# shenyunhang/NA-fWebSOD

Measured on AMD Instinct MI355X. Metric: images/sec (600px, 2000 proposals) VGG16-C5 WSDDN fwd+bwd, higher is better.
Workload: dtype f32 (2xf16 split, 3-pass f16 MFMA, fp32 accumulate)

## Files before the change

### include/naws.h

```cpp
#ifndef NAWS_H_
#define NAWS_H_

#include <stdint.h>

#ifdef __cplusplus
extern "C" {
#endif

#define NAWS_OK 0
#define NAWS_ERR_SHAPE (-1)
#define NAWS_ERR_ARG (-2)
#define NAWS_ERR_NULL (-3)
#define NAWS_ERR_LAUNCH (-4)
#define NAWS_ERR_UNSUPPORTED (-5)

#define NAWS_LAYOUT_NCHW 0
#define NAWS_LAYOUT_NHWC 1

const char* naws_version(void);
int naws_last_hip_error(void);


int naws_conv3x3_c3_nchw_to_nhwc_fwd(const float* X, const float* Wt, const float* bias,
                                     int N, int H, int W, int Cout, int relu,
                                     float* Y, void* stream);

int naws_conv3x3_pack_weight(const float* W_oihw, int Cout, int Cin, float* W_packed,
                             void* stream);

int naws_conv3x3_nhwc_fwd(const float* X, const float* Wp, const float* bias,
                          int N, int H, int W, int Cin, int Cout, int dilation, int relu,
                          float* Y, void* stream);

int64_t naws_winograd_workspace_floats(int N, int H, int W, int Cin, int Cout, int dilation);
int naws_winograd_weight_transform(const float* W_oihw, int Cout, int Cin, float* U,
                                   void* stream);
int naws_conv3x3_winograd_nhwc_fwd(const float* X, const float* U, const float* bias,
                                   int N, int H, int W, int Cin, int Cout, int dilation, int relu,
                                   float* workspace, float* Y, void* stream);

int naws_maxpool2x2_nhwc_fwd(const float* X, int N, int H, int W, int C, int stride,
                             float* Y, void* stream);

int naws_maxpool3x3_nhwc_fwd(const float* X, int N, int H, int W, int C, int stride,
                             float* Y, void* stream);

int naws_nchw_to_nhwc(const float* X, int N, int C, int H, int W, float* Y, void* stream);
int naws_nhwc_to_nchw(const float* X, int N, int H, int W, int C, float* Y, void* stream);
// ... 417 lines not shown
```

### na-fwebsod_amd/csrc/misc_ops.hip

```cpp
#include <float.h>
#include <math.h>
#include "naws_common.h"

thread_local int g_naws_last_hip_error = 0;

extern "C" const char* naws_version(void) { return "naws-hip 0.1 (gfx950)"; }
extern "C" int naws_last_hip_error(void) { return g_naws_last_hip_error; }

#include <atomic>
#include <mutex>
#include <string.h>
namespace {
constexpr int LDS_SLOTS = 512;
constexpr int MAX_DEV = 256;
struct LdsSlot {
  std::atomic<const void*> kernel;
  std::atomic<unsigned long long> dev[MAX_DEV / 64];
};
LdsSlot g_lds_slots[LDS_SLOTS];
std::mutex g_lds_mutex;
std::atomic<int> g_knobs[NAWS_KNOB_COUNT] = {{0}, {0}, {0}, {11}, {0}, {42}, {0}, {0}, {0}};
const char* const g_knob_names[NAWS_KNOB_COUNT] = {"gemm", "x3", "h2", "conv_ring", "conv_bn",
                                                    "roi_nw", "wino", "split", "sgd_wgs"};
}

int naws_allow_lds_impl(const void* kernel, int bytes) {
  int dev = 0;
  if (hipGetDevice(&dev) != hipSuccess) return naws_check_launch();
  const bool in_range = dev >= 0 && dev < MAX_DEV;
  const size_t h0 = ((uintptr_t)kernel >> 4) % LDS_SLOTS;
  if (in_range) {
    size_t h = h0;
    for (int probe = 0; probe < LDS_SLOTS; ++probe, h = (h + 1) % LDS_SLOTS) {
      const void* k = g_lds_slots[h].kernel.load(std::memory_order_acquire);
      if (k == kernel) {
        if ((g_lds_slots[h].dev[dev >> 6].load(std::memory_order_acquire) >> (dev & 63)) & 1ULL)
          return NAWS_OK;
        break;
      }
      if (k == nullptr) break;
    }
  }
  std::lock_guard<std::mutex> lock(g_lds_mutex);
  LdsSlot* slot = nullptr;
  if (in_range) {
    size_t h = h0;
// ... 161 lines not shown
#pragma unroll
    for (int k = 0; k < 27; ++k) {
      const float v = in[k];
      const float* wr = wl + k * Cout + g * OC_PER;
#pragma unroll
      for (int o = 0; o < OC_PER; ++o) acc[o] = fmaf(v, wr[o], acc[o]);
    }
    float* out = Y + pix * Cout + g * OC_PER;
#pragma unroll
    for (int o = 0; o < OC_PER; o += 4) {
      float4 r;
      r.x = acc[o + 0] + bl[g * OC_PER + o + 0];
      r.y = acc[o + 1] + bl[g * OC_PER + o + 1];
      r.z = acc[o + 2] + bl[g * OC_PER + o + 2];
      r.w = acc[o + 3] + bl[g * OC_PER + o + 3];
      if (relu) { r.x = fmaxf(r.x, 0.f); r.y = fmaxf(r.y, 0.f); r.z = fmaxf(r.z, 0.f); r.w = fmaxf(r.w, 0.f); }
      *reinterpret_cast<float4*>(out + o) = r;
    }
  }
}


constexpr int C3_TW = 64, C3_TH = 8, C3_STRIP = 32, C3_LD = C3_TW + 4;
__global__ __launch_bounds__(256) void conv_c3_tile_kernel(const float* __restrict__ X,
                                                           const float* __restrict__ Wt,
                                                           const float* __restrict__ bias, int H,
                                                           int W, int relu, float* __restrict__ Y) {
  __shared__ float tile[3][C3_TH + 2][C3_LD];
  __shared__ __attribute__((aligned(16))) float wl[27][64];
  const int x0 = blockIdx.x * C3_TW, y0 = blockIdx.y * C3_TH, n = blockIdx.z;
  const float* Xn = X + (int64_t)n * 3 * H * W;
  for (int i = threadIdx.x; i < 3 * (C3_TH + 2) * (C3_TW + 2); i += 256) {
    const int col = i % (C3_TW + 2);
    const int r = (i / (C3_TW + 2)) % (C3_TH + 2);
    const int c = i / ((C3_TW + 2) * (C3_TH + 2));
    const int yy = y0 + r - 1, xx = x0 + col - 1;
    const bool ok = (yy >= 0) && (yy < H) && (xx >= 0) && (xx < W);
    const int yc = min(max(yy, 0), H - 1), xc = min(max(xx, 0), W - 1);
    const float v = Xn[((int64_t)c * H + yc) * W + xc];
    tile[c][r][col] = ok ? v : 0.f;
  }
  for (int i = threadIdx.x; i < 27 * 64; i += 256) wl[i % 27][i / 27] = Wt[i];
  __syncthreads();
  const int q = threadIdx.x & 15, grp = threadIdx.x >> 4;
  const int row = grp & 7, strip = grp >> 3;
  float w[27][4];
#pragma unroll
  for (int k = 0; k < 27; ++k) {
    const float4 t = *reinterpret_cast<const float4*>(&wl[k][4 * q]);
    w[k][0] = t.x; w[k][1] = t.y; w[k][2] = t.z; w[k][3] = t.w;
  }
  float4 bv = make_float4(0.f, 0.f, 0.f, 0.f);
  if (bias) bv = *reinterpret_cast<const float4*>(bias + 4 * q);
  const int y = y0 + row;
  const int cx = strip * C3_STRIP;
  float win[3][3][3];
#pragma unroll
  for (int c = 0; c < 3; ++c)
#pragma unroll
    for (int kh = 0; kh < 3; ++kh) {
      win[c][kh][0] = tile[c][row + kh][cx];
      win[c][kh][1] = tile[c][row + kh][cx + 1];
    }
  float* yrow = Y + (((int64_t)n * H + y) * W + x0 + cx) * 64 + 4 * q;
#pragma unroll
  for (int i = 0; i < C3_STRIP; ++i) {
// ... 33 lines not shown

__global__ __launch_bounds__(TB) void maxpool2_kernel(const float4* __restrict__ X, int N, int H,
                                                      int W, int C4, int stride, int Ho, int Wo,
                                                      float4* __restrict__ Y) {
  const int64_t total = (int64_t)N * Ho * Wo * C4;
  for (int64_t t = (int64_t)blockIdx.x * TB + threadIdx.x; t < total;
       t += (int64_t)gridDim.x * TB) {
    const int c = (int)(t % C4);
    const int xo = (int)((t / C4) % Wo);
    const int yo = (int)((t / ((int64_t)C4 * Wo)) % Ho);
    const int n = (int)(t / ((int64_t)C4 * Wo * Ho));
    const int y = yo * stride, x = xo * stride;
    const float4* p = X + (((int64_t)n * H + y) * W + x) * C4 + c;
    const float4 a = p[0], b = p[C4], d = p[(int64_t)W * C4], e = p[(int64_t)W * C4 + C4];
    float4 r;
    r.x = fmaxf(fmaxf(a.x, b.x), fmaxf(d.x, e.x));
    r.y = fmaxf(fmaxf(a.y, b.y), fmaxf(d.y, e.y));
    r.z = fmaxf(fmaxf(a.z, b.z), fmaxf(d.z, e.z));
    r.w = fmaxf(fmaxf(a.w, b.w), fmaxf(d.w, e.w));
    Y[t] = r;
  }
}

__global__ void transpose_batched_kernel(const float* __restrict__ X, int rows, int cols,
                                         float* __restrict__ Y) {
  __shared__ float tile[32][33];
  const int64_t boff = (int64_t)blockIdx.z * rows * cols;
  const int c0 = blockIdx.x * 32, r0 = blockIdx.y * 32;
  for (int i = threadIdx.y; i < 32; i += blockDim.y) {
    const int r = r0 + i, c = c0 + threadIdx.x;
    if (r < rows && c < cols) tile[i][threadIdx.x] = X[boff + (int64_t)r * cols + c];
  }
  __syncthreads();
  for (int i = threadIdx.y; i < 32; i += blockDim.y) {
    const int c = c0 + i, r = r0 + threadIdx.x;
    if (r < rows && c < cols) Y[boff + (int64_t)c * rows + r] = tile[threadIdx.x][i];
  }
}

__global__ void unary_kernel(int op, const float* __restrict__ X, int64_t n, float a, float b,
                             float* __restrict__ Y) {
  for (int64_t i = (int64_t)blockIdx.x * blockDim.x + threadIdx.x; i < n;
       i += (int64_t)gridDim.x * blockDim.x) {
    const float x = X[i];
    float y;
    switch (op) {
// ... 123 lines not shown
}

__global__ void dropout_mask_kernel(uint64_t seed, uint32_t thr, int64_t n,
                                    float* __restrict__ mask) {
  for (int64_t i = (int64_t)blockIdx.x * blockDim.x + threadIdx.x; i < n;
       i += (int64_t)gridDim.x * blockDim.x)
    mask[i] = naws_keep(seed, (uint64_t)i, thr) ? 1.0f : 0.0f;
}

inline int grid_for(int64_t n, int tb = TB, int cap = 256 * 8) {
  return (int)std::min<int64_t>(std::max<int64_t>(naws_cdiv(n, tb), 1), cap);
}

}

extern "C" int naws_conv3x3_c3_nchw_to_nhwc_fwd(const float* X, const float* Wt,
                                                const float* bias, int N, int H, int W, int Cout,
                                                int relu, float* Y, void* stream) {
  if (N <= 0 || H <= 0 || W <= 0 || Cout <= 0) return NAWS_ERR_SHAPE;
  if (Cout % 16 != 0 || ((uintptr_t)Y % 16) != 0) return NAWS_ERR_ARG;
  NAWS_REQUIRE_PTR(X); NAWS_REQUIRE_PTR(Wt); NAWS_REQUIRE_PTR(Y);
  if (Cout == 64 && N <= 65535 && naws_cdiv(H, C3_TH) <= 65535) {
    dim3 grid((unsigned)naws_cdiv(W, C3_TW), (unsigned)naws_cdiv(H, C3_TH), (unsigned)N);
    hipLaunchKernelGGL(conv_c3_tile_kernel, grid, dim3(256), 0, (hipStream_t)stream, X, Wt, bias,
                       H, W, relu, Y);
    return naws_check_launch();
  }
  const size_t lds = (size_t)(27 + 1) * Cout * sizeof(float);
  const int64_t total = (int64_t)N * H * W * (Cout / 16);
  hipLaunchKernelGGL(conv_c3_kernel<16>, dim3(grid_for(total, TB, 256 * 16)), dim3(TB), lds,
                     (hipStream_t)stream, X, Wt, bias, N, H, W, Cout, relu, Y);
  return naws_check_launch();
}

extern "C" int naws_conv3x3_pack_weight(const float* W_oihw, int Cout, int Cin, float* W_packed,
                                        void* stream) {
  if (Cout <= 0 || Cin <= 0) return NAWS_ERR_SHAPE;
  NAWS_REQUIRE_PTR(W_oihw); NAWS_REQUIRE_PTR(W_packed);
  hipLaunchKernelGGL(pack_weight_kernel, dim3(grid_for((int64_t)Cout * Cin * 9)), dim3(TB), 0,
                     (hipStream_t)stream, W_oihw, Cout, Cin, W_packed);
  return naws_check_launch();
}

extern "C" int naws_maxpool2x2_nhwc_fwd(const float* X, int N, int H, int W, int C, int stride,
                                        float* Y, void* stream) {
  if (N <= 0 || H < 2 || W < 2 || C <= 0) return NAWS_ERR_SHAPE;
  if (stride != 1 && stride != 2) return NAWS_ERR_ARG;
  if (C % 4 != 0 || (((uintptr_t)X | (uintptr_t)Y) % 16) != 0) return NAWS_ERR_ARG;
  NAWS_REQUIRE_PTR(X); NAWS_REQUIRE_PTR(Y);
  const int Ho = (H - 2) / stride + 1, Wo = (W - 2) / stride + 1;
  const int64_t total = (int64_t)N * Ho * Wo * (C / 4);
  hipLaunchKernelGGL(maxpool2_kernel, dim3(grid_for(total, TB, 256 * 16)), dim3(TB), 0,
                     (hipStream_t)stream, (const float4*)X, N, H, W, C / 4, stride, Ho, Wo,
                     (float4*)Y);
  return naws_check_launch();
}

static int transpose_batched(const float* X, int batch, int rows, int cols, float* Y,
                             void* stream) {
  if (batch <= 0 || rows <= 0 || cols <= 0) return NAWS_ERR_SHAPE;
  NAWS_REQUIRE_PTR(X); NAWS_REQUIRE_PTR(Y);
  if (batch > 65535 || naws_cdiv(rows, 32) > 65535) return NAWS_ERR_UNSUPPORTED;
  dim3 grid((unsigned)naws_cdiv(cols, 32), (unsigned)naws_cdiv(rows, 32), batch);
  hipLaunchKernelGGL(transpose_batched_kernel, grid, dim3(32, 8), 0, (hipStream_t)stream, X,
                     rows, cols, Y);
  return naws_check_launch();
}

extern "C" int naws_nchw_to_nhwc(const float* X, int N, int C, int H, int W, float* Y,
                                 void* stream) {
  if (H <= 0 || W <= 0) return NAWS_ERR_SHAPE;
  return transpose_batched(X, N, C, H * W, Y, stream);
}
// ... 184 lines not shown
```

### na-fwebsod_amd/csrc/naws_common.h

```cpp
#pragma once
#include <hip/hip_runtime.h>
#include <stdint.h>
#include <algorithm>
#include "naws.h"

#define NAWS_WAVE 64

extern thread_local int g_naws_last_hip_error;

static inline int naws_check_launch() {
  hipError_t e = hipGetLastError();
  if (e != hipSuccess) {
    g_naws_last_hip_error = (int)e;
    return NAWS_ERR_LAUNCH;
  }
  return NAWS_OK;
}

int naws_allow_lds_impl(const void* kernel, int bytes);
template <typename K>
static inline int naws_allow_lds(K kernel, int bytes = 160 * 1024) {
  return naws_allow_lds_impl(reinterpret_cast<const void*>(kernel), bytes);
}

int naws_wino_col_gemm_impl(int P, int Cout, int Cin, const void* V2, const float* invV,
                            const void* U2, const float* scaleU, float* S, hipStream_t stream);

enum NawsKnob { NAWS_KNOB_GEMM = 0, NAWS_KNOB_X3, NAWS_KNOB_H2, NAWS_KNOB_CONV_RING,
                NAWS_KNOB_CONV_BN, NAWS_KNOB_ROI_NW, NAWS_KNOB_WINO, NAWS_KNOB_SPLIT, NAWS_KNOB_SGD_WGS,
                NAWS_KNOB_COUNT };
int naws_knob(int knob);

#define NAWS_REQUIRE_PTR(p) \
  do {                      \
    if ((p) == nullptr) return NAWS_ERR_NULL; \
  } while (0)

static inline int64_t naws_cdiv(int64_t a, int64_t b) { return (a + b - 1) / b; }

__device__ __forceinline__ float wave_sum(float v) {
#pragma unroll
  for (int o = 32; o > 0; o >>= 1) v += __shfl_xor(v, o, 64);
  return v;
}
__device__ __forceinline__ float wave_max(float v) {
#pragma unroll
  for (int o = 32; o > 0; o >>= 1) v = fmaxf(v, __shfl_xor(v, o, 64));
  return v;
}

__device__ __host__ __forceinline__ uint32_t naws_hash_u32(uint64_t seed, uint64_t idx) {
  uint64_t z = seed + 0x9E3779B97F4A7C15ull * (idx + 1);
// ... 185 lines not shown
```

### na-fwebsod_amd/csrc/roi_ops.hip

```cpp
#include <float.h>
#include <stdlib.h>
#include "naws_common.h"

namespace {

struct RoiBins {
  int batch, start_w, start_h, roi_w, roi_h;
};

__device__ __forceinline__ RoiBins roi_frame(const float* roi, float spatial_scale) {
  RoiBins b;
  b.batch = (int)roi[0];
  int start_w = (int)roundf(roi[1] * spatial_scale);
  int start_h = (int)roundf(roi[2] * spatial_scale);
  int end_w = (int)roundf(roi[3] * spatial_scale);
  int end_h = (int)roundf(roi[4] * spatial_scale);
  b.start_w = start_w;
  b.start_h = start_h;
  b.roi_w = max(end_w - start_w + 1, 1);
  b.roi_h = max(end_h - start_h + 1, 1);
  return b;
}

__device__ __forceinline__ void bin_range(int p, float bin_size, int roi_start, int limit,
// ... 338 lines not shown
  unsigned short* dst = Q + pl * plane_out;
  for (int u = threadIdx.x; u < 512; u += 256) {
    const int hh = u & 1, i = (u >> 1) & 15, sl = u >> 5;
    const int slab = k0 / 16 + sl;
    uint4 v = make_uint4(0u, 0u, 0u, 0u);
    if (slab * 16 < K && r0 + i < R)
      v = *reinterpret_cast<const uint4*>(src + ((long long)slab * R + r0 + i) * 16 + hh * 8);
    unsigned short* d = &t[sl][i][hh * 8];
    d[0] = v.x & 0xffff; d[1] = v.x >> 16; d[2] = v.y & 0xffff; d[3] = v.y >> 16;
    d[4] = v.z & 0xffff; d[5] = v.z >> 16; d[6] = v.w & 0xffff; d[7] = v.w >> 16;
  }
  __syncthreads();
  const int k = k0 + threadIdx.x;
  if (k >= K) return;
  const int sl = threadIdx.x >> 4, kk = threadIdx.x & 15;
  unsigned w[8];
#pragma unroll
  for (int i = 0; i < 8; ++i) w[i] = t[sl][2 * i][kk] | ((unsigned)t[sl][2 * i + 1][kk] << 16);
  unsigned short* o = dst + ((long long)blockIdx.y * K + k) * 16;
  *reinterpret_cast<uint4*>(o) = make_uint4(w[0], w[1], w[2], w[3]);
  *reinterpret_cast<uint4*>(o + 8) = make_uint4(w[4], w[5], w[6], w[7]);
}

template <int STEP>
__global__ __launch_bounds__(256) void roi_maxmap_kernel(const float* __restrict__ S, int H, int W,
                                                         int C, float* __restrict__ D,
                                                         long long total4) {
  const long long i = (long long)blockIdx.x * 256 + threadIdx.x;
  if (i >= total4) return;
  const int c4 = C / 4;
  const int cq = (int)(i % c4);
  const long long pix = i / c4;
  const int x = (int)(pix % W), y = (int)((pix / W) % H);
  const int dy = (y + STEP < H) ? STEP : 0, dx = (x + STEP < W) ? STEP : 0;
  const float* base = S + (pix * C + cq * 4);
  const float4 v00 = *reinterpret_cast<const float4*>(base);
  const float4 v01 = *reinterpret_cast<const float4*>(base + (long long)dx * C);
  const float4 v10 = *reinterpret_cast<const float4*>(base + (long long)dy * W * C);
  const float4 v11 = *reinterpret_cast<const float4*>(base + ((long long)dy * W + dx) * C);
  float4 m = make_float4(-FLT_MAX, -FLT_MAX, -FLT_MAX, -FLT_MAX);
#define NAWS_MX(b, v) \
  b.x = (v.x > b.x) ? v.x : b.x; b.y = (v.y > b.y) ? v.y : b.y; \
  b.z = (v.z > b.z) ? v.z : b.z; b.w = (v.w > b.w) ? v.w : b.w;
  NAWS_MX(m, v00) NAWS_MX(m, v01) NAWS_MX(m, v10) NAWS_MX(m, v11)
#undef NAWS_MX
  *reinterpret_cast<float4*>(D + (pix * C + cq * 4)) = m;
// ... 123 lines not shown
  const long long K = (long long)C * pooled_h * pooled_w;
  if (C % 64 != 0 || pooled_h * pooled_w > 256 || K % 32 != 0 || (int64_t)R * (C / 64) >= 0x7fffffffLL)
    return NAWS_ERR_UNSUPPORTED;
  if ((((uintptr_t)X | (uintptr_t)planes) & 15) != 0) return NAWS_ERR_ARG;
  RoiPlaneOut po;
  po.P = (unsigned short*)planes; po.inv_scale = scales + R; po.amax_words = (const unsigned*)amax_words;
  po.n_words = n_words; po.plane = K * R; po.R = R; po.bf16 = 0;
  hipLaunchKernelGGL(roi_pool_nhwc_xcd_kernel<true>, dim3((unsigned)(R * (C / 64))), dim3(64),
                     (size_t)(64 * pooled_h * pooled_w + 1) * sizeof(float), (hipStream_t)stream, X, C,
                     H, W, rois, R, boost, pooled_h, pooled_w, spatial_scale, C / 64, (float*)nullptr,
                     po);
  return naws_check_launch();
}

extern "C" int64_t naws_roi_pool_workspace_floats(int N, int C, int H, int W) {
  if (N <= 0 || C <= 0 || H <= 0 || W <= 0) return 0;
  return (int64_t)2 * N * H * W * C;
}

static int roi_maxmaps(const float* X, int N, int C, int H, int W, float* M2, float* M4,
                       hipStream_t s) {
  const long long total4 = (long long)N * H * W * (C / 4);
  if (naws_cdiv(total4, 256) > 0x7fffffffLL) return NAWS_ERR_UNSUPPORTED;
  hipLaunchKernelGGL(roi_maxmap_kernel<1>, dim3((unsigned)naws_cdiv(total4, 256)), dim3(256), 0, s, X, H,
                     W, C, M2, total4);
  hipLaunchKernelGGL(roi_maxmap_kernel<2>, dim3((unsigned)naws_cdiv(total4, 256)), dim3(256), 0, s,
                     (const float*)M2, H, W, C, M4, total4);
  return naws_check_launch();
}

extern "C" int naws_roi_pool_f_nhwc_hier_fwd(const float* X, int N, int C, int H, int W,
                                             const float* rois, int R, const float* boost,
                                             int pooled_h, int pooled_w, float spatial_scale,
                                             float* workspace, float* Y, void* stream) {
  if (R < 0 || N <= 0 || C <= 0 || H <= 0 || W <= 0 || pooled_h <= 0 || pooled_w <= 0)
    return NAWS_ERR_SHAPE;
  if (R == 0) return NAWS_OK;
  NAWS_REQUIRE_PTR(X); NAWS_REQUIRE_PTR(rois); NAWS_REQUIRE_PTR(Y); NAWS_REQUIRE_PTR(workspace);
  if (C % 64 != 0 || pooled_h * pooled_w > 256 || (int64_t)R * (C / 64) >= 0x7fffffffLL)
    return NAWS_ERR_UNSUPPORTED;
  if ((((uintptr_t)X | (uintptr_t)workspace) & 15) != 0) return NAWS_ERR_ARG;
  hipStream_t s = (hipStream_t)stream;
  const int rc = roi_maxmaps(X, N, C, H, W, workspace, workspace + (long long)N * H * W * C, s);
  if (rc != NAWS_OK) return rc;
  hipLaunchKernelGGL((roi_pool_nhwc_xcd_kernel<false, true, 4>), dim3((unsigned)(R * (C / 64))), dim3(256),
                     (size_t)(64 * pooled_h * pooled_w + 1) * sizeof(float), s, X, C, H, W, rois, R,
// ... 425 lines not shown
```

### na-fwebsod_amd/naws_hip/engine.py

```python

import collections
import contextlib
import os

import numpy as np
import torch

from . import head_arith
from . import lib as L
from . import ops
from .planes import ALL, FcPlanes
from .reducer import ArenaReducer, message_slice, owner_pieces
from .update import HIDDEN, UpdateSchedule

VGG16_CONVS = [
    ('conv1_1', 3, 64, 1), ('conv1_2', 64, 64, 1), ('pool', 2),
    ('conv2_1', 64, 128, 1), ('conv2_2', 128, 128, 1), ('pool', 2),
    ('conv3_1', 128, 256, 1), ('conv3_2', 256, 256, 1), ('conv3_3', 256, 256, 1), ('pool', 2),
    ('conv4_1', 256, 512, 1), ('conv4_2', 512, 512, 1), ('conv4_3', 512, 512, 1), ('pool4',),
    ('conv5_1', 512, 512, None), ('conv5_2', 512, 512, None), ('conv5_3', 512, 512, None),
]

ConvStep = collections.namedtuple('ConvStep',
                                  'name form cin cout dilation direct_alt pool2 weight_bound')
# ... 180 lines not shown
            wd.append(w)
        if any(e % 4 for e in ends):
            raise NotImplementedError('SGD hyper-parameter runs must end on multiples of 4 floats')
        self._seg_host = (list(ends), list(lr_mult), list(wd))
        self.seg_end = torch.tensor(ends, dtype=torch.int64, device=device)
        self.seg_lr_mult = torch.tensor(lr_mult, dtype=torch.float32, device=device)
        self.seg_wd = torch.tensor(wd, dtype=torch.float32, device=device)
        self.lr = torch.zeros((1,), dtype=torch.float32, device=device)
        self._lr_host = 0.0
        self.sgd_iter_count = 0
        self.step_count = 0
        self.conv_layers = []
        self.stat_state = None
        self.conv_streams = True
        self.fused_planes = True
        self.fuse_wgrad_update = True
        self.defer_update = None
        self.DIRECT_MIN_TILES = 256
        self.WINO_F4_MIN_CIN = 256
        self.FC8_KSPLIT = 4
        self.UPDATE_AFTER = max(1, ar.update_after)
        self._update_behind_heads = ar.update_after > 0
        self.ROI_POOL_ON_CHAINS = True
        self._fc8_ws = None
        self._seg_ring = None
        self._amax5 = None
        self._streams = []
        self._fc = None
        self._planes_dirty = True
        for kv in filter(None, os.environ.get('NAWS_ENGINE_SET', '').split(',')):
            k, v = kv.split('=')
            if not (k.isupper() and isinstance(getattr(self, k, None), int)):
                raise ValueError('NAWS_ENGINE_SET: %r is not an integer engine choice' % k)
            setattr(self, k, int(v))

    def blob(self, name):
        self.flush()
        self._planes_dirty = True
        return self.arena.view(self.params, name)

    def blob_ro(self, name):
        self.flush()
        return self.arena.view(self.params, name)

    def _one_hyper_run(self, start, count):
        ends = self._seg_host[0]
# ... 83 lines not shown
                    out['planes_' + k], out['scales_' + k] = v.planes, v.scales
                else:
                    out['planes_' + k] = v
        return out

    def set_update_route(self, pipeline_update=None, sharded_update=False):
        self.sched.set_route(pipeline_update, sharded_update)

    def export_blobs(self, with_momentum=True):
        self.flush()
        if with_momentum and not self.sched.mom_synced:
            raise RuntimeError('NAWS.SHARDED_UPDATE: fc6_w momentum rows live with their owners; '
                               'call gather_sharded_state() on EVERY rank before a checkpoint')
        out = {}
        for lay in self.conv_layers:
            if lay.w is not None:
                out[lay.step.name + '_w'], out[lay.step.name + '_b'] = lay.w, lay.b
        for name, _ in self.arena.specs:
            out[name] = self.blob_ro(name)
            if with_momentum:
                out[name + '_momentum'] = self.momentum_blob(name)
        return out

    def _conv_chain(self, layers, st, out=None, amax_out=None):
        x, bound, aff, pooled = st
        words = (torch.zeros((len(layers),), device=self.device, dtype=torch.int32)
                 if any(lay.step.form in _H2_FORMS for lay in layers) else None)
        for k, lay in enumerate(layers):
            s = lay.step
            if s.form == 'pool3':
                x = ops.maxpool3x3_nhwc(x, s.stride)
                continue
            if s.form == 'pool':
                if not pooled:
                    x = ops.maxpool2x2_nhwc(x, s.stride)
                pooled = False
                continue
            form, w, b, d = s.form, lay.operand, lay.b, s.dilation
            if lay.direct is not None:
                tiles = x.shape[0] * ((x.shape[1] + 7) // 8) * ((x.shape[2] + 31) // 32)
                if tiles * (s.cout // 128) >= self.DIRECT_MIN_TILES:
                    form, w = 'h2_direct', lay.direct
            if aff != _IDENTITY and form != 'h2_direct':
                raise ValueError('%s: its input bound carries (mul, add) = %r, which the %s form '
                                 'cannot apply' % (s.name, aff, form))
            last = k == len(layers) - 1
            dst = out if last else None
            pooled = s.pool2 and form in ('h2_direct', 'x3_direct', 'bf16_wp')
            word, word_aff = None, _IDENTITY
            if form in _H2_FORMS:
                word = amax_out if last and amax_out is not None else words[k:k + 1]
            if form == 'c3':
                y = ops.conv3x3_c3_nchw_to_nhwc(x, w, b, True)
                if lay.affine is not None:
                    word, word_aff = ops.amax_word(x), lay.affine
                x = y
            elif form == 'h2_direct':
                x = ops.conv3x3_nhwc_f16x2(x, w, b, True, out=dst, amax_in=bound, in_mul=aff[0],
                                           in_add=aff[1], amax_out=word, pool2=pooled,
                                           amax_out_zeroed=word is not amax_out, dilation=d)
            elif form in ('h2_wino2', 'h2_wino4'):
                x = ops.conv3x3_winograd_nhwc_f16x2(x, w, b, d, True, out=dst, amax_in=bound,
                                                    amax_out=word)
            elif form == 'x3_direct':
                x = ops.conv3x3_nhwc_f32x3(x, w, b, d, True, out=dst, pool2=pooled)
            elif form == 'x3_wino':
                x = ops.conv3x3_winograd_nhwc_f32x3(x, w, b, d, True, out=dst)
            elif form == 'f32_direct':
                x = ops.conv3x3_nhwc(x, w, b, d, True, out=dst)
            elif form == 'f32_wino':
                x = ops.conv3x3_winograd_nhwc(x, w, b, d, True, out=dst)
            elif form == 'bf16_wp':
                x = ops.conv3x3_nhwc_bf16_wp(x, w, b, d, True, out=dst, pool2=pooled)
            bound, aff = word, word_aff
        return ChainState(x, bound, aff, pooled)

    def conv_body(self, data, roi_job=None):
        n = data.shape[0]
        planes = self.conv_layers[-1].step.form in _H2_FORMS
# ... 1 lines not shown
        self._roi_maps = None
        self._roi_operand = None
        self._amax5 = (torch.empty((n if per_image else 1,), device=self.device,
                                   dtype=torch.int32) if planes else None)
        split = self.sched.waits_for_heads(per_image and self._update_behind_heads)
        if not per_image:
            res = self._conv_chain(self.conv_layers, ChainState(data, None, _IDENTITY, False),
                                   amax_out=self._amax5).x
            self._roi_maps_of = (res.data_ptr(), res._version)
            return res
        h, w = data.shape[2], data.shape[3]
        for s in (lay.step for lay in self.conv_layers if lay.step.form in _POOL_FORMS):
            h, w = pooled_size(s, h, w)
        out = torch.empty((n, h, w, 512), device=self.device, dtype=torch.float32)
        self._roi_maps = ((torch.empty_like(out), torch.empty_like(out))
                          if self.arith.roi_maps_on_chains else None)
        self._roi_maps_of = (out.data_ptr(), out._version)
        pooled = None
        if (roi_job is not None and planes and self.ROI_POOL_ON_CHAINS
                and roi_job[0].shape[0] > 0 and len(roi_job[2]) == n + 1):
            self._check_rows_grouped_by_image(roi_job[0], roi_job[2])
            pooled = ops.roi_pool_operand(roi_job[0].shape[0], self.k6, self.device)
        main = torch.cuda.current_stream(self.device)
        start = main.record_event()
        while len(self._streams) < n:
            self._streams.append(side_stream(self.device, 'conv%d' % len(self._streams)))
        chains = [ChainState(data[i:i + 1], None, _IDENTITY, False) for i in range(n)]
        layers = self.conv_layers
        if split:
            ua = min(max(1, self.UPDATE_AFTER), len(layers) - 1)
            evs = []
            for i in range(n):
                st = self._streams[i]
                st.wait_event(start)
                with torch.cuda.stream(st):
                    chains[i] = self._conv_chain(layers[:ua], chains[i])
                    evs.append(st.record_event())
            self.sched.launch(evs)
            layers = layers[ua:]
        for i in range(n):
            st = self._streams[i]
            if not split:
                st.wait_event(start)
            with torch.cuda.stream(st):
                af = None if self._amax5 is None else self._amax5[i:i + 1]
                self._conv_chain(layers, chains[i], out=out[i:i + 1], amax_out=af)
                if self._roi_maps is not None:
                    ops.roi_maxmaps(out[i:i + 1], self._roi_maps[0][i:i + 1], self._roi_maps[1][i:i + 1])
                    if pooled is not None and roi_job[2][i + 1] > roi_job[2][i]:
                        ops.roi_pool_f_f16x2_range(out, roi_job[0], self._amax5, pooled, roi_job[2][i],
                                                   roi_job[2][i + 1], self._roi_maps, self.roi_size,
                                                   self.roi_size, self.spatial_scale,
                                                   boost=roi_job[1].reshape(-1))
                done = st.record_event()
            main.wait_event(done)
        if pooled is not None:
            self._roi_operand = (pooled, out.data_ptr(), self._roi_job_key(roi_job[0], roi_job[1]))
        return out

    @staticmethod
    def _roi_job_key(rois, obn_scores):
        return (rois.data_ptr(), rois._version, obn_scores.data_ptr(), obn_scores._version)

    def _check_rows_grouped_by_image(self, rois, seg):
        import os
        if os.environ.get('NAWS_DEBUG_CHECKS') != '1':
            return
        want = torch.repeat_interleave(
            torch.arange(len(seg) - 1, device=rois.device, dtype=rois.dtype),
# ... 439 lines not shown
```

### na-fwebsod_amd/naws_hip/lib.py

```python
import ctypes as C
import os

_HERE = os.path.dirname(os.path.abspath(__file__))
LIB_PATH = os.environ.get('NAWS_LIB') or os.path.join(os.path.dirname(_HERE), 'lib',
                                                       'libnaws_hip.so')
_ENV_KNOBS = {'NAWS_GEMM_VARIANT': 'gemm', 'NAWS_X3_VARIANT': 'x3', 'NAWS_H2_VARIANT': 'h2',
              'NAWS_CONV_RING': 'conv_ring', 'NAWS_CONV_BN': 'conv_bn', 'NAWS_ROI_NW': 'roi_nw',
              'NAWS_WINO_VARIANT': 'wino', 'NAWS_SPLIT': 'split', 'NAWS_SGD_WGS': 'sgd_wgs'}

OK, ERR_SHAPE, ERR_ARG, ERR_NULL, ERR_LAUNCH, ERR_UNSUPPORTED = 0, -1, -2, -3, -4, -5
_ERR_NAMES = {
    ERR_SHAPE: 'NAWS_ERR_SHAPE', ERR_ARG: 'NAWS_ERR_ARG', ERR_NULL: 'NAWS_ERR_NULL',
    ERR_LAUNCH: 'NAWS_ERR_LAUNCH', ERR_UNSUPPORTED: 'NAWS_ERR_UNSUPPORTED',
}
LAYOUT_NCHW, LAYOUT_NHWC = 0, 1
EPI_NONE, EPI_BIAS, EPI_BIAS_RELU, EPI_BIAS_RELU_DROP, EPI_GATE_POS = range(5)
UN_LOG, UN_SCALE, UN_REPLACE_NAN, UN_LEAKY_RELU, UN_CLIP, UN_RELU = range(6)
BIN_ADD, BIN_SUB, BIN_MUL, BIN_DIV, BIN_GATE_POS = range(5)
PLANES_F16X2, PLANES_BF16X3, PLANES_BF16 = range(3)

p, i32, i64, u64, f32 = C.c_void_p, C.c_int, C.c_int64, C.c_uint64, C.c_float

PROTOTYPES = {
    'naws_conv3x3_c3_nchw_to_nhwc_fwd': [p, p, p, i32, i32, i32, i32, i32, p, p],
    'naws_conv3x3_pack_weight': [p, i32, i32, p, p],
    'naws_conv3x3_nhwc_fwd': [p, p, p, i32, i32, i32, i32, i32, i32, i32, p, p],
    'naws_maxpool2x2_nhwc_fwd': [p, i32, i32, i32, i32, i32, p, p],
    'naws_maxpool2x2_nhwc_bwd': [p, p, p, i32, i32, i32, i32, i32, p, p],
    'naws_maxpool3x3_nhwc_fwd': [p, i32, i32, i32, i32, i32, p, p],
    'naws_conv2d_pack_weight': [p, i32, i32, i32, p, p],
    'naws_conv2d_nhwc_fwd': [p, p, p, i32, i32, i32, i32, i32, i32, i32, i32, i32, i32, p, p],
    'naws_affine_channel_fwd': [p, p, p, i32, i32, i64, i32, p, p],
    'naws_conv3x3_dgrad_pack_weight': [p, i32, i32, p, p],
    'naws_conv3x3_nhwc_wgrad': [p, p, i32, i32, i32, i32, i32, i32, p, p, p, p],
    'naws_roi_pool_f_bwd': [p, p, p, i32, i32, i32, i32, i32, i32, i32, i32, p, p],
    'naws_winograd_weight_transform': [p, i32, i32, p, p],
    'naws_conv3x3_winograd_nhwc_fwd': [p, p, p, i32, i32, i32, i32, i32, i32, i32, p, p, p],
    'naws_nchw_to_nhwc': [p, i32, i32, i32, i32, p, p],
    'naws_nhwc_to_nchw': [p, i32, i32, i32, i32, p, p],
    'naws_roi_pool_f_fwd': [p, i32, i32, i32, i32, i32, p, i32, p, i32, i32, f32, p, p, p],
    'naws_roi_align_fwd': [p, i32, i32, i32, i32, p, i32, i32, i32, f32, i32, p, p],
    'naws_roi_align_bwd': [p, p, i32, i32, i32, i32, i32, i32, i32, f32, i32, p, p],
    'naws_roi_context_fwd': [p, i32, f32, i32, i32, p, p, p],
    'naws_roi_loop_pool_fwd': [p, i32, i32, i32, i32, i32, p, i32, p, i32, i32, f32, p, p, p],
    'naws_roi_feature_boost_fwd': [p, p, i32, i32, p, p],
    'naws_roi_feature_boost_bwd': [p, p, i32, i32, p, p],
    'naws_roi_iou_fwd': [p, i32, p, p],
# ... 182 lines not shown
```

### na-fwebsod_amd/naws_hip/ops.py

```python
import ctypes as C

import numpy as np
import torch

from . import lib as L

_f32 = torch.float32


def _stream():
    return torch.cuda.current_stream().cuda_stream


def _chk(t, name, dtype=_f32):
    if not isinstance(t, torch.Tensor) or not t.is_cuda:
        raise TypeError('%s must be a HIP device tensor (the naws ops have no CPU path)' % name)
    if t.dtype != dtype:
        raise TypeError('%s must be %s, got %s' % (name, dtype, t.dtype))
    if not t.is_contiguous():
        raise ValueError('%s must be contiguous' % name)
    return t


def _ptr(t):
    return 0 if t is None else t.data_ptr()


def _workspace(workspace, need, device, sizer, dtype=_f32):
    if workspace is None:
        return torch.empty((max(int(need), 4),), device=device, dtype=dtype)
    if (not isinstance(workspace, torch.Tensor) or not workspace.is_cuda
            or workspace.dtype != dtype or workspace.numel() < need
            or not workspace.is_contiguous()):
        raise TypeError('workspace: contiguous %s on the device, >= %s' % (dtype, sizer))
    return workspace


def conv3x3_c3_nchw_to_nhwc(x, w_oihw, bias, relu=True, out=None):
    _chk(x, 'x'); _chk(w_oihw, 'w')
    n, c, h, w = x.shape
    assert c == 3 and tuple(w_oihw.shape[1:]) == (3, 3, 3)
    cout = w_oihw.shape[0]
    y = out if out is not None else torch.empty((n, h, w, cout), device=x.device, dtype=_f32)
    L.call('naws_conv3x3_c3_nchw_to_nhwc_fwd', x.data_ptr(), w_oihw.data_ptr(), _ptr(bias),
           n, h, w, cout, int(relu), y.data_ptr(), _stream())
    return y


def conv3x3_pack_weight(w_oihw):
    _chk(w_oihw, 'w')
    cout, cin = w_oihw.shape[:2]
    wp = torch.empty((cout, 3, 3, cin), device=w_oihw.device, dtype=_f32)
    L.call('naws_conv3x3_pack_weight', w_oihw.data_ptr(), cout, cin, wp.data_ptr(), _stream())
    return wp


def conv3x3_nhwc(x, w_packed, bias, dilation=1, relu=True, out=None):
    _chk(x, 'x'); _chk(w_packed, 'w_packed')
    n, h, w, cin = x.shape
    cout = w_packed.shape[0]
    y = out if out is not None else torch.empty((n, h, w, cout), device=x.device, dtype=_f32)
    L.call('naws_conv3x3_nhwc_fwd', x.data_ptr(), w_packed.data_ptr(), _ptr(bias), n, h, w, cin,
           cout, dilation, int(relu), y.data_ptr(), _stream())
    return y


# ... 1713 lines not shown
```

Measured before the change: 166.8.

## Fuse ROI max-map passes, add row-sliding stride-1 maxpool, optional conv1 amax fusion

```diff
diff --git a/include/naws.h b/include/naws.h
--- a/include/naws.h
+++ b/include/naws.h
@@ -24,6 +24,9 @@
 int naws_conv3x3_c3_nchw_to_nhwc_fwd(const float* X, const float* Wt, const float* bias,
                                      int N, int H, int W, int Cout, int relu,
                                      float* Y, void* stream);
+int naws_conv3x3_c3_nchw_to_nhwc_amax_fwd(const float* X, const float* Wt, const float* bias,
+                                          int N, int H, int W, int Cout, int relu, float* Y,
+                                          uint32_t* amax_in, int amax_stride, void* stream);
 
 int naws_conv3x3_pack_weight(const float* W_oihw, int Cout, int Cin, float* W_packed,
                              void* stream);
diff --git a/na-fwebsod_amd/csrc/misc_ops.hip b/na-fwebsod_amd/csrc/misc_ops.hip
--- a/na-fwebsod_amd/csrc/misc_ops.hip
+++ b/na-fwebsod_amd/csrc/misc_ops.hip
@@ -19,9 +19,10 @@
 };
 LdsSlot g_lds_slots[LDS_SLOTS];
 std::mutex g_lds_mutex;
-std::atomic<int> g_knobs[NAWS_KNOB_COUNT] = {{0}, {0}, {0}, {11}, {0}, {42}, {0}, {0}, {0}};
+std::atomic<int> g_knobs[NAWS_KNOB_COUNT] = {{0}, {0}, {0}, {11}, {0}, {42}, {0}, {0}, {0}, {0}};
 const char* const g_knob_names[NAWS_KNOB_COUNT] = {"gemm", "x3", "h2", "conv_ring", "conv_bn",
-                                                    "roi_nw", "wino", "split", "sgd_wgs"};
+                                                    "roi_nw", "wino", "split", "sgd_wgs",
+                                                    "roi_maps"};
 }
 
 int naws_allow_lds_impl(const void* kernel, int bytes) {
@@ -229,14 +230,19 @@
 
 
 constexpr int C3_TW = 64, C3_TH = 8, C3_STRIP = 32, C3_LD = C3_TW + 4;
+template <bool AMAX>
 __global__ __launch_bounds__(256) void conv_c3_tile_kernel(const float* __restrict__ X,
                                                            const float* __restrict__ Wt,
                                                            const float* __restrict__ bias, int H,
-                                                           int W, int relu, float* __restrict__ Y) {
+                                                           int W, int relu, float* __restrict__ Y,
+                                                           unsigned* __restrict__ amax_in,
+                                                           int amax_stride) {
   __shared__ float tile[3][C3_TH + 2][C3_LD];
   __shared__ __attribute__((aligned(16))) float wl[27][64];
+  __shared__ float red[4];
   const int x0 = blockIdx.x * C3_TW, y0 = blockIdx.y * C3_TH, n = blockIdx.z;
   const float* Xn = X + (int64_t)n * 3 * H * W;
+  float am = 0.f;
   for (int i = threadIdx.x; i < 3 * (C3_TH + 2) * (C3_TW + 2); i += 256) {
     const int col = i % (C3_TW + 2);
     const int r = (i / (C3_TW + 2)) % (C3_TH + 2);
@@ -246,9 +252,20 @@
     const int yc = min(max(yy, 0), H - 1), xc = min(max(xx, 0), W - 1);
     const float v = Xn[((int64_t)c * H + yc) * W + xc];
     tile[c][r][col] = ok ? v : 0.f;
+    if (AMAX && ok && r >= 1 && r <= C3_TH && col >= 1 && col <= C3_TW) am = fmaxf(am, fabsf(v));
   }
   for (int i = threadIdx.x; i < 27 * 64; i += 256) wl[i % 27][i / 27] = Wt[i];
+  if (AMAX) {
+#pragma unroll
+    for (int d = 32; d > 0; d >>= 1) am = fmaxf(am, __shfl_xor(am, d));
+    if ((threadIdx.x & 63) == 0) red[threadIdx.x >> 6] = am;
+  }
   __syncthreads();
+  if (AMAX && threadIdx.x == 0) {
+    unsigned* word = amax_in + (int64_t)n * amax_stride;
+    const unsigned v = __float_as_uint(fmaxf(fmaxf(red[0], red[1]), fmaxf(red[2], red[3])));
+    if (v > __hip_atomic_load(word, __ATOMIC_RELAXED, __HIP_MEMORY_SCOPE_AGENT)) atomicMax(word, v);
+  }
   const int q = threadIdx.x & 15, grp = threadIdx.x >> 4;
   const int row = grp & 7, strip = grp >> 3;
   float w[27][4];
@@ -328,6 +345,36 @@
   }
 }
 
+template <int RS>
+__global__ __launch_bounds__(TB) void maxpool2_s1_kernel(const float4* __restrict__ X, int H, int W,
+                                                         int C4, int Ho, int Wo, int nseg,
+                                                         int64_t total, float4* __restrict__ Y) {
+  const int64_t t = (int64_t)blockIdx.x * TB + threadIdx.x;
+  if (t >= total) return;
+  const int c = (int)(t % C4);
+  const int xo = (int)((t / C4) % Wo);
+  const int seg = (int)((t / ((int64_t)C4 * Wo)) % nseg);
+  const int64_t n = t / ((int64_t)C4 * Wo * nseg);
+  const int y0 = seg * RS;
+  const float4* p = X + ((n * H + y0) * W + xo) * C4 + c;
+  float4* q = Y + ((n * Ho + y0) * Wo + xo) * C4 + c;
+  float4 prev;
+#pragma unroll
+  for (int k = 0; k <= RS; ++k) {
+    const int64_t ro = (int64_t)min(k, H - 1 - y0) * W * C4;
+    const float4 a = p[ro], b = p[ro + C4];
+    float4 h;
+    h.x = fmaxf(a.x, b.x); h.y = fmaxf(a.y, b.y); h.z = fmaxf(a.z, b.z); h.w = fmaxf(a.w, b.w);
+    if (k > 0 && y0 + k < H) {
+      float4 r;
+      r.x = fmaxf(prev.x, h.x); r.y = fmaxf(prev.y, h.y);
+      r.z = fmaxf(prev.z, h.z); r.w = fmaxf(prev.w, h.w);
+      q[(int64_t)(k - 1) * Wo * C4] = r;
+    }
+    prev = h;
+  }
+}
+
 __global__ void transpose_batched_kernel(const float* __restrict__ X, int rows, int cols,
                                          float* __restrict__ Y) {
   __shared__ float tile[32][33];
@@ -497,14 +544,30 @@
   NAWS_REQUIRE_PTR(X); NAWS_REQUIRE_PTR(Wt); NAWS_REQUIRE_PTR(Y);
   if (Cout == 64 && N <= 65535 && naws_cdiv(H, C3_TH) <= 65535) {
     dim3 grid((unsigned)naws_cdiv(W, C3_TW), (unsigned)naws_cdiv(H, C3_TH), (unsigned)N);
-    hipLaunchKernelGGL(conv_c3_tile_kernel, grid, dim3(256), 0, (hipStream_t)stream, X, Wt, bias,
-                       H, W, relu, Y);
+    hipLaunchKernelGGL(conv_c3_tile_kernel<false>, grid, dim3(256), 0, (hipStream_t)stream, X, Wt,
+                       bias, H, W, relu, Y, (unsigned*)nullptr, 0);
     return naws_check_launch();
   }
   const size_t lds = (size_t)(27 + 1) * Cout * sizeof(float);
   const int64_t total = (int64_t)N * H * W * (Cout / 16);
   hipLaunchKernelGGL(conv_c3_kernel<16>, dim3(grid_for(total, TB, 256 * 16)), dim3(TB), lds,
                      (hipStream_t)stream, X, Wt, bias, N, H, W, Cout, relu, Y);
+  return naws_check_launch();
+}
+
+extern "C" int naws_conv3x3_c3_nchw_to_nhwc_amax_fwd(const float* X, const float* Wt,
+                                                     const float* bias, int N, int H, int W,
+                                                     int Cout, int relu, float* Y,
+                                                     uint32_t* amax_in, int amax_stride,
+                                                     void* stream) {
+  if (N <= 0 || H <= 0 || W <= 0) return NAWS_ERR_SHAPE;
+  if (Cout != 64 || N > 65535 || naws_cdiv(H, C3_TH) > 65535) return NAWS_ERR_UNSUPPORTED;
+  if (((uintptr_t)Y % 16) != 0 || ((uintptr_t)amax_in % 4) != 0 || amax_stride < 0)
+    return NAWS_ERR_ARG;
+  NAWS_REQUIRE_PTR(X); NAWS_REQUIRE_PTR(Wt); NAWS_REQUIRE_PTR(Y); NAWS_REQUIRE_PTR(amax_in);
+  dim3 grid((unsigned)naws_cdiv(W, C3_TW), (unsigned)naws_cdiv(H, C3_TH), (unsigned)N);
+  hipLaunchKernelGGL(conv_c3_tile_kernel<true>, grid, dim3(256), 0, (hipStream_t)stream, X, Wt,
+                     bias, H, W, relu, Y, (unsigned*)amax_in, amax_stride);
   return naws_check_launch();
 }
 
@@ -524,6 +587,16 @@
   if (C % 4 != 0 || (((uintptr_t)X | (uintptr_t)Y) % 16) != 0) return NAWS_ERR_ARG;
   NAWS_REQUIRE_PTR(X); NAWS_REQUIRE_PTR(Y);
   const int Ho = (H - 2) / stride + 1, Wo = (W - 2) / stride + 1;
+  if (stride == 1) {
+    constexpr int RS = 8;
+    const int nseg = (int)naws_cdiv(Ho, RS);
+    const int64_t items = (int64_t)N * nseg * Wo * (C / 4);
+    if (naws_cdiv(items, TB) > 0x7fffffffLL) return NAWS_ERR_UNSUPPORTED;
+    hipLaunchKernelGGL(maxpool2_s1_kernel<RS>, dim3((unsigned)naws_cdiv(items, TB)), dim3(TB), 0,
+                       (hipStream_t)stream, (const float4*)X, H, W, C / 4, Ho, Wo, nseg, items,
+                       (float4*)Y);
+    return naws_check_launch();
+  }
   const int64_t total = (int64_t)N * Ho * Wo * (C / 4);
   hipLaunchKernelGGL(maxpool2_kernel, dim3(grid_for(total, TB, 256 * 16)), dim3(TB), 0,
                      (hipStream_t)stream, (const float4*)X, N, H, W, C / 4, stride, Ho, Wo,
diff --git a/na-fwebsod_amd/csrc/naws_common.h b/na-fwebsod_amd/csrc/naws_common.h
--- a/na-fwebsod_amd/csrc/naws_common.h
+++ b/na-fwebsod_amd/csrc/naws_common.h
@@ -28,6 +28,7 @@
 
 enum NawsKnob { NAWS_KNOB_GEMM = 0, NAWS_KNOB_X3, NAWS_KNOB_H2, NAWS_KNOB_CONV_RING,
                 NAWS_KNOB_CONV_BN, NAWS_KNOB_ROI_NW, NAWS_KNOB_WINO, NAWS_KNOB_SPLIT, NAWS_KNOB_SGD_WGS,
+                NAWS_KNOB_ROI_MAPS,
                 NAWS_KNOB_COUNT };
 int naws_knob(int knob);
 
diff --git a/na-fwebsod_amd/csrc/roi_ops.hip b/na-fwebsod_amd/csrc/roi_ops.hip
--- a/na-fwebsod_amd/csrc/roi_ops.hip
+++ b/na-fwebsod_amd/csrc/roi_ops.hip
@@ -384,6 +384,63 @@
   *reinterpret_cast<uint4*>(o + 8) = make_uint4(w[4], w[5], w[6], w[7]);
 }
 
+template <int RS>
+__global__ __launch_bounds__(256) void roi_maxmaps_kernel(const float* __restrict__ X, int H, int W,
+                                                          int C, int nseg, float* __restrict__ M2,
+                                                          float* __restrict__ M4,
+                                                          long long total4) {
+  const long long i = (long long)blockIdx.x * 256 + threadIdx.x;
+  if (i >= total4) return;
+  const int c4 = C / 4;
+  const int cq = (int)(i % c4);
+  long long t = i / c4;
+  const int x = (int)(t % W);
+  t /= W;
+  const int seg = (int)(t % nseg);
+  const long long n = t / nseg;
+  const int y0 = seg * RS;
+  const long long rowC = (long long)W * C;
+  const float* col = X + n * H * rowC + (long long)x * C + cq * 4;
+  const int d1 = min(1, W - 1 - x) * C, d2 = min(2, W - 1 - x) * C, d3 = min(3, W - 1 - x) * C;
+  const long long obase = (n * H * W + x) * (long long)C + cq * 4;
+#define NAWS_MX(b, v) \
+  b.x = (v.x > b.x) ? v.x : b.x; b.y = (v.y > b.y) ? v.y : b.y; \
+  b.z = (v.z > b.z) ? v.z : b.z; b.w = (v.w > b.w) ? v.w : b.w;
+  const float4 low = make_float4(-FLT_MAX, -FLT_MAX, -FLT_MAX, -FLT_MAX);
+  float4 h2[2], h4[4];
+#pragma unroll
+  for (int k = 0; k < RS + 3; ++k) {
+    const float* p = col + (long long)min(y0 + k, H - 1) * rowC;
+    const float4 a = *reinterpret_cast<const float4*>(p);
+    const float4 b = *reinterpret_cast<const float4*>(p + d1);
+    const float4 c = *reinterpret_cast<const float4*>(p + d2);
+    const float4 d = *reinterpret_cast<const float4*>(p + d3);
+    float4 m = low;
+    NAWS_MX(m, a) NAWS_MX(m, b)
+    h2[k % 2] = m;
+    NAWS_MX(m, c) NAWS_MX(m, d)
+    h4[k % 4] = m;
+    if (k >= 3) {
+      const int y = y0 + k - 3;
+      if (y < H) {
+        float4 m4 = low;
+        NAWS_MX(m4, h4[(k - 3) % 4]) NAWS_MX(m4, h4[(k - 2) % 4])
+        NAWS_MX(m4, h4[(k - 1) % 4]) NAWS_MX(m4, h4[k % 4])
+        *reinterpret_cast<float4*>(M4 + obase + y * rowC) = m4;
+      }
+    }
+    if (k >= 1 && k <= RS) {
+      const int y = y0 + k - 1;
+      if (y < H) {
+        float4 m2 = low;
+        NAWS_MX(m2, h2[(k - 1) % 2]) NAWS_MX(m2, h2[k % 2])
+        *reinterpret_cast<float4*>(M2 + obase + y * rowC) = m2;
+      }
+    }
+  }
+#undef NAWS_MX
+}
+
 template <int STEP>
 __global__ __launch_bounds__(256) void roi_maxmap_kernel(const float* __restrict__ S, int H, int W,
                                                          int C, float* __restrict__ D,
@@ -553,6 +610,14 @@
                        hipStream_t s) {
   const long long total4 = (long long)N * H * W * (C / 4);
   if (naws_cdiv(total4, 256) > 0x7fffffffLL) return NAWS_ERR_UNSUPPORTED;
+  if (naws_knob(NAWS_KNOB_ROI_MAPS) != 2) {
+    constexpr int RS = 8;
+    const int nseg = (int)naws_cdiv(H, RS);
+    const long long items = (long long)N * nseg * W * (C / 4);
+    hipLaunchKernelGGL(roi_maxmaps_kernel<RS>, dim3((unsigned)naws_cdiv(items, 256)), dim3(256), 0, s,
+                       X, H, W, C, nseg, M2, M4, items);
+    return naws_check_launch();
+  }
   hipLaunchKernelGGL(roi_maxmap_kernel<1>, dim3((unsigned)naws_cdiv(total4, 256)), dim3(256), 0, s, X, H,
                      W, C, M2, total4);
   hipLaunchKernelGGL(roi_maxmap_kernel<2>, dim3((unsigned)naws_cdiv(total4, 256)), dim3(256), 0, s,
diff --git a/na-fwebsod_amd/naws_hip/engine.py b/na-fwebsod_amd/naws_hip/engine.py
--- a/na-fwebsod_amd/naws_hip/engine.py
+++ b/na-fwebsod_amd/naws_hip/engine.py
@@ -226,6 +226,7 @@
         self.UPDATE_AFTER = max(1, ar.update_after)
         self._update_behind_heads = ar.update_after > 0
         self.ROI_POOL_ON_CHAINS = True
+        self.CONV1_AMAX_FUSED = False
         self._fc8_ws = None
         self._seg_ring = None
         self._amax5 = None
@@ -355,10 +356,14 @@
                 out[name + '_momentum'] = self.momentum_blob(name)
         return out
 
-    def _conv_chain(self, layers, st, out=None, amax_out=None):
+    def _hands_on_word(self, lay):
+        return lay.step.form in _H2_FORMS or (
+            lay.step.form == 'c3' and lay.affine is not None and self.CONV1_AMAX_FUSED)
+
+    def _conv_chain(self, layers, st, out=None, amax_out=None, words=None):
         x, bound, aff, pooled = st
-        words = (torch.zeros((len(layers),), device=self.device, dtype=torch.int32)
-                 if any(lay.step.form in _H2_FORMS for lay in layers) else None)
+        if words is None and any(self._hands_on_word(lay) for lay in layers):
+            words = torch.zeros((len(layers),), device=self.device, dtype=torch.int32)
         for k, lay in enumerate(layers):
             s = lay.step
             if s.form == 'pool3':
@@ -384,10 +389,14 @@
             if form in _H2_FORMS:
                 word = amax_out if last and amax_out is not None else words[k:k + 1]
             if form == 'c3':
-                y = ops.conv3x3_c3_nchw_to_nhwc(x, w, b, True)
-                if lay.affine is not None:
-                    word, word_aff = ops.amax_word(x), lay.affine
-                x = y
+                if lay.affine is not None and self.CONV1_AMAX_FUSED:
+                    word, word_aff = words[k:k + 1], lay.affine
+                    x = ops.conv3x3_c3_nchw_to_nhwc(x, w, b, True, amax_in=word)
+                else:
+                    y = ops.conv3x3_c3_nchw_to_nhwc(x, w, b, True)
+                    if lay.affine is not None:
+                        word, word_aff = ops.amax_word(x), lay.affine
+                    x = y
             elif form == 'h2_direct':
                 x = ops.conv3x3_nhwc_f16x2(x, w, b, True, out=dst, amax_in=bound, in_mul=aff[0],
                                            in_add=aff[1], amax_out=word, pool2=pooled,
@@ -435,11 +444,16 @@
             self._check_rows_grouped_by_image(roi_job[0], roi_job[2])
             pooled = ops.roi_pool_operand(roi_job[0].shape[0], self.k6, self.device)
         main = torch.cuda.current_stream(self.device)
+        layers = self.conv_layers
         start = main.record_event()
         while len(self._streams) < n:
             self._streams.append(side_stream(self.device, 'conv%d' % len(self._streams)))
         chains = [ChainState(data[i:i + 1], None, _IDENTITY, False) for i in range(n)]
-        layers = self.conv_layers
+        wd = [None] * n
+        if any(self._hands_on_word(lay) for lay in layers):
+            for i in range(n):
+                with torch.cuda.stream(self._streams[i]):
+                    wd[i] = torch.zeros((len(layers),), device=self.device, dtype=torch.int32)
         if split:
             ua = min(max(1, self.UPDATE_AFTER), len(layers) - 1)
             evs = []
@@ -447,17 +461,19 @@
                 st = self._streams[i]
                 st.wait_event(start)
                 with torch.cuda.stream(st):
-                    chains[i] = self._conv_chain(layers[:ua], chains[i])
+                    chains[i] = self._conv_chain(layers[:ua], chains[i],
+                                                 words=None if wd[i] is None else wd[i][:ua])
                     evs.append(st.record_event())
             self.sched.launch(evs)
             layers = layers[ua:]
+            wd = [None if v is None else v[ua:] for v in wd]
         for i in range(n):
             st = self._streams[i]
             if not split:
                 st.wait_event(start)
             with torch.cuda.stream(st):
                 af = None if self._amax5 is None else self._amax5[i:i + 1]
-                self._conv_chain(layers, chains[i], out=out[i:i + 1], amax_out=af)
+                self._conv_chain(layers, chains[i], out=out[i:i + 1], amax_out=af, words=wd[i])
                 if self._roi_maps is not None:
                     ops.roi_maxmaps(out[i:i + 1], self._roi_maps[0][i:i + 1], self._roi_maps[1][i:i + 1])
                     if pooled is not None and roi_job[2][i + 1] > roi_job[2][i]:
diff --git a/na-fwebsod_amd/naws_hip/lib.py b/na-fwebsod_amd/naws_hip/lib.py
--- a/na-fwebsod_amd/naws_hip/lib.py
+++ b/na-fwebsod_amd/naws_hip/lib.py
@@ -6,7 +6,8 @@
                                                        'libnaws_hip.so')
 _ENV_KNOBS = {'NAWS_GEMM_VARIANT': 'gemm', 'NAWS_X3_VARIANT': 'x3', 'NAWS_H2_VARIANT': 'h2',
               'NAWS_CONV_RING': 'conv_ring', 'NAWS_CONV_BN': 'conv_bn', 'NAWS_ROI_NW': 'roi_nw',
-              'NAWS_WINO_VARIANT': 'wino', 'NAWS_SPLIT': 'split', 'NAWS_SGD_WGS': 'sgd_wgs'}
+              'NAWS_WINO_VARIANT': 'wino', 'NAWS_SPLIT': 'split', 'NAWS_SGD_WGS': 'sgd_wgs',
+              'NAWS_ROI_MAPS': 'roi_maps'}
 
 OK, ERR_SHAPE, ERR_ARG, ERR_NULL, ERR_LAUNCH, ERR_UNSUPPORTED = 0, -1, -2, -3, -4, -5
 _ERR_NAMES = {
@@ -23,6 +24,7 @@
 
 PROTOTYPES = {
     'naws_conv3x3_c3_nchw_to_nhwc_fwd': [p, p, p, i32, i32, i32, i32, i32, p, p],
+    'naws_conv3x3_c3_nchw_to_nhwc_amax_fwd': [p, p, p, i32, i32, i32, i32, i32, p, p, i32, p],
     'naws_conv3x3_pack_weight': [p, i32, i32, p, p],
     'naws_conv3x3_nhwc_fwd': [p, p, p, i32, i32, i32, i32, i32, i32, i32, p, p],
     'naws_maxpool2x2_nhwc_fwd': [p, i32, i32, i32, i32, i32, p, p],
diff --git a/na-fwebsod_amd/naws_hip/ops.py b/na-fwebsod_amd/naws_hip/ops.py
--- a/na-fwebsod_amd/naws_hip/ops.py
+++ b/na-fwebsod_amd/naws_hip/ops.py
@@ -36,12 +36,20 @@
     return workspace
 
 
-def conv3x3_c3_nchw_to_nhwc(x, w_oihw, bias, relu=True, out=None):
+def conv3x3_c3_nchw_to_nhwc(x, w_oihw, bias, relu=True, out=None, amax_in=None):
     _chk(x, 'x'); _chk(w_oihw, 'w')
     n, c, h, w = x.shape
     assert c == 3 and tuple(w_oihw.shape[1:]) == (3, 3, 3)
     cout = w_oihw.shape[0]
     y = out if out is not None else torch.empty((n, h, w, cout), device=x.device, dtype=_f32)
+    if amax_in is not None:
+        if (amax_in.dtype != torch.int32 or not amax_in.is_contiguous()
+                or amax_in.numel() not in (1, n)):
+            raise TypeError('amax_in must be a contiguous int32 tensor of 1 or %d words' % n)
+        L.call('naws_conv3x3_c3_nchw_to_nhwc_amax_fwd', x.data_ptr(), w_oihw.data_ptr(),
+               _ptr(bias), n, h, w, cout, int(relu), y.data_ptr(), amax_in.data_ptr(),
+               0 if amax_in.numel() == 1 else 1, _stream())
+        return y
     L.call('naws_conv3x3_c3_nchw_to_nhwc_fwd', x.data_ptr(), w_oihw.data_ptr(), _ptr(bias),
            n, h, w, cout, int(relu), y.data_ptr(), _stream())
     return y
```

Result: no change. 166.3 (-0.3%).
